# beer-asr/beer

Hardware: AMD Instinct MI355X
Metric: frames/sec per VB iteration (E+M) (higher is better)
Workload: dtype f32

## Files before the change

### beer_amd/csrc/estep_bf16.hip

```cpp

#include <cstdlib>
#include <type_traits>
#include <utility>

#include "estep_mfma.h"
#include "estep_tiles.h"

#ifndef BEER_K1_ABL
#define BEER_K1_ABL 0
#endif
#ifndef BEER_K2_ABL
#define BEER_K2_ABL 0
#endif
#ifndef BEER_AF_ABL
#define BEER_AF_ABL 0
#endif
#ifndef BEER_AFI_ABL
#define BEER_AFI_ABL 0
#endif
#ifndef BEER_LNFI_ABL
#define BEER_LNFI_ABL 0
#endif
#ifndef BEER_LNFI_SLEEP
#define BEER_LNFI_SLEEP 0
// ... 45 lines not shown
    else
        asm volatile("v_mfma_f32_16x16x32_bf16 %0, %1, %2, %0" : "+v"(acc) : "v"(a), "v"(b));
}
__device__ __forceinline__ void mfma_drain() {
    asm volatile("s_nop 15\n\ts_nop 15" ::: "memory");
    __builtin_amdgcn_sched_barrier(0);
}

__host__ __device__ inline size_t frame_image_tile_u4(int nk_used, int nqt) {
    return (size_t)(nk_used * NP * 2 + nqt * NP) * 64;
}
__host__ __device__ constexpr int img_nqt(int nk_used) { return nk_used <= 3 ? 5 : 6; }
constexpr int kImgMaxNK = 4;
__host__ __device__ inline int stat_slab(int j) { return j + j / 7; }
__host__ __device__ inline int nk16_of(int cov, int D) {
    return ((nslab_of(cov, D) + 7) / 8 + 1) / 2 * 2;
}
__host__ __device__ inline int ld16_of(int D) {
    const int ld = 4 * d4_of(D) + 8;
    return (ld / 4) % 2 ? ld : ld + 4;
}
constexpr float kConstEps = 5.9604644775390625e-8f;
constexpr int kBlockU4 = NP * 64;

__device__ inline double entry_value(int cov, int D, int K, int k, int slab, int e,
                                     const float* __restrict__ row, bool* is_const) {
    const int D4 = d4_of(D), Dp = 4 * D4, nslab = nslab_of(cov, D);
    *is_const = false;
    if (slab >= nslab) return 0.0;
    const int t = slab_entry(cov, D, slab);
    const int a = t & 0xff, b = ((t >> 8) & 0xff) + e, sq = t >> 16;
    if (a == Dp && b - e == Dp) {
        *is_const = true;
        return 0.0;
    }
    if (k >= K) return 0.0;
    if (sq) return b < D ? -0.5 * (double)row[cov == BEER_ISO ? D : D + b] : 0.0;
    if (a < D) {
        if (b >= D || b < a) return 0.0;
        return b == a ? -0.5 * (double)row[D + a * D + a]
                      : -0.5 * ((double)row[D + a * D + b] + (double)row[D + b * D + a]);
    }
    return b < D ? (double)row[b] : 0.0;
}
// ... 15 lines not shown

__global__ __launch_bounds__(256) void packx_kernel(int cov, int D, int K, int NT,
                                                    const float* __restrict__ E,
                                                    const float* __restrict__ logw,
                                                    unsigned short* __restrict__ P,
                                                    int* __restrict__ tab, int G, int Gp,
                                                    const float* __restrict__ c0, int lane_major) {
    extern __shared__ __attribute__((aligned(16))) char pack_lds[];
    const int nk = nk16_of(cov, D), nent = nk * 32;
    const int slot = blockIdx.x;
    const int k = slot % Gp < G ? (slot / Gp) * G + slot % Gp : K;
    const int chunk = slot / (NT * 16), kk = slot % (NT * 16);
    const int c = lane_major ? kk % NT : 4 * (kk / 64) + (kk % 4);
    const int i = lane_major ? kk / NT : (kk % 64) / 4;
    if (slot == 0)
        for (int s = threadIdx.x; s < (nk + 1) * 8; s += blockDim.x) {
            const int Dp = 4 * d4_of(D);
            tab[s] = s < nslab_of(cov, D) ? slab_entry(cov, D, s) : ((Dp + 2) | ((Dp + 4) << 8));
        }
    const int Qs = stats_dim(cov, D);
    float* rowl = reinterpret_cast<float*>(pack_lds);
    if (k < K)
        for (int q = threadIdx.x; q < Qs; q += blockDim.x) rowl[q] = E[(size_t)k * Qs + q];
    __syncthreads();
    unsigned short* base = P + ((size_t)chunk * nk * NT) * (NP * 512);
    auto put = [&](int q, float v) {
        const int s = q / 32, g = (q % 32) / 8, j = q % 8;
        unsigned short* dst = base + ((size_t)s * NT + c) * (NP * 512) + (g * 16 + i) * 8 + j;
        unsigned short p[3];
        split3_scalar(v, p);
        dst[0] = p[0];
        dst[512] = p[1];
        dst[1024] = p[2];
    };
    const int nslab = nslab_of(cov, D);
    for (int q = threadIdx.x; q < nent; q += blockDim.x) {
        bool is_const;
        const double v = entry_value(cov, D, K, k, q / 4, q % 4, rowl, &is_const);
        if (!is_const) {
            put(q, (float)v);
        } else if (q % 4 == 0) {
            const bool last = q / 4 == nslab - 1;
            const double want = k < K ? const_share(cov, D, q / 4, rowl, logw ? (double)logw[k] : 0.0) -
                                            (last ? (double)c0[0] : 0.0)
                                      : (last ? kPadLogit : 0.0);
            const float hi = (float)want;
            const double rem = (want - (double)hi) * (1.0 / (double)kConstEps);
            put(q, hi);
            put(q + 1, (rem == rem && fabs(rem) < 1.0e30) ? (float)rem : 0.f);
            put(q + 2, 0.f);
// ... 59 lines not shown
        }
    }
}

template <int NT, int MT, int GQ, bool PACKED, bool SQ, bool LNO, bool IMG = false, bool BL = false>
__global__ __launch_bounds__(kThreads, MT * NT <= 32 ? 2 : 1) void llhx_kernel(
    int64_t nframes, int D, int K, int S, int G, int gl, int jw, int nk,
    const float* __restrict__ X, const u4* __restrict__ Pall, const int* __restrict__ tab,
    float* __restrict__ resps, float* __restrict__ log_norm, double* __restrict__ llh_sum,
    float* __restrict__ xt_out, int xt_floats, int nku, int cg, const float* __restrict__ c0,
    const u4* __restrict__ img = nullptr) {
    static_assert(!IMG || (MT == 2 && !PACKED && LNO), "the image holds 32-frame tiles");
    static_assert(!BL || (NT == 16 && MT == 2 && !IMG), "half k-steps of 8 tiles, hipcc-scheduled form");
    extern __shared__ __attribute__((aligned(16))) char smem[];
    const int LD = ld16_of(D);
    const int tid = threadIdx.x, lane = tid & 63;
    const int wave = __builtin_amdgcn_readfirstlane(tid >> 6);
    const int i = lane & 15, g = lane >> 4;
    constexpr int FW = 16 * MT, NW = kThreads / 64;
    constexpr bool PIN = MT * NT > 32;
    float* xw = reinterpret_cast<float*>(smem) + wave * (FW * LD);
    int* tabs = reinterpret_cast<int*>(reinterpret_cast<float*>(smem) + NW * FW * LD);
    constexpr int kHalfBytes = 8 * kBlockU4 * 16;
    char* ring = smem + (((size_t)NW * FW * LD * sizeof(float) + (size_t)(nk + 1) * 8 * sizeof(int)
                          + 1023) & ~(size_t)1023);
    int64_t bx = blockIdx.x;
    int by = 0;
    {
        const int nch = (K + 16 * NT - 1) / (16 * NT);
        constexpr int FBK = FW * NW;
// ... 29 lines not shown
    for (int m = 0; m < MT; ++m)
#pragma unroll
        for (int c = 0; c < NT; ++c) acc[m][c] = f32x4{0, 0, 0, 0};

    const float* xrow[MT];
#pragma unroll
    for (int m = 0; m < MT; ++m) xrow[m] = xw + (m * 16 + i) * LD;

    const int kbase = by * (16 * NT);
    const u4* Pl = Pall + (size_t)by * nk * NT * kBlockU4 + lane;
    const int* tl = tabs + 2 * g;

    struct AFrag { u4 w[NP][MT]; };
    auto make_half = [&](int s, int m, int h, AFrag& f) {
        const int t = tl[8 * s + h];
        const int a = t & 0xff, j = (t >> 8) & 0xff;
        const bool sq = SQ && (t >> 16) != 0;
        const f32x4 bb = *reinterpret_cast<const f32x4*>(xrow[m] + j);
        const float xx = xrow[m][a];
        f32x4 p;
#pragma unroll
        for (int e = 0; e < 4; ++e) p[e] = bb[e] * (sq ? bb[e] : xx);
#pragma unroll
        for (int e = 0; e < 2; ++e) {
            unsigned w3[3];
            split3(p[2 * e], p[2 * e + 1], w3);
#pragma unroll
            for (int q = 0; q < NP; ++q) f.w[q][m][2 * h + e] = w3[q];
        }
    };
    constexpr int BT = 2, NBATCH = NT / BT;
    static_assert(NT % BT == 0 && NBATCH % 2 == 0, "B batches alternate between two buffers");
    struct BFrag { u4 p[BT][NP]; };
    auto load_b = [&](int64_t blk, BFrag& b) {
#pragma unroll
        for (int c = 0; c < BT; ++c)
#pragma unroll
// ... 17 lines not shown
#pragma unroll
        for (int n = 0; n < kHalfBytes / 1024 / NW; ++n)
            __builtin_amdgcn_global_load_lds(reinterpret_cast<const u4*>(src + n * (NW * 1024)),
                                             (lds_ptr)(dst + n * (NW * 1024)), 16, 0, 0);
    };
    auto publish = [&]() {
        asm volatile("s_waitcnt vmcnt(0) lgkmcnt(0)" ::: "memory");
        __builtin_amdgcn_s_barrier();
    };
    auto batch = [&](int s, int bi, const AFrag& cur, AFrag& nxt, const BFrag& b, BFrag& bn) {
        if constexpr (PIN) {
            static_assert(!PIN || (MT * 2 == NBATCH && 6 * BT * MT == 48), "one half fragment per batch");
            const int hm = bi % MT, hh = bi / MT;
            const int64_t blk = (int64_t)s * NT + (bi + 1) * BT;
            int t = 0;
            f32x4 bb = {0.f, 0.f, 0.f, 0.f}, p = {0.f, 0.f, 0.f, 0.f};
            float xx = 0.f;
            Split3Steps st[2];
#pragma unroll
            for (int n = 0; n < 48; ++n) {
                const int pr = n / (BT * MT), c = (n / MT) % BT, m = n % MT;
                mfma_bf16_pinned<false>(acc[m][bi * BT + c], cur.w[kProdA[pr]][m],
                                        b.p[c][kProdB[pr]]);
                if (BEER_K1_ABL >= 1 && n >= NP * BT) {
                } else if (BEER_K1_ABL >= 2) {
                } else if (n < NP * BT) {
#ifdef BEER_K1_FAKEB
                    bn.p[n / NP][n % NP] = Pl[(size_t)((blk + n / NP) & 3) * kBlockU4 + 64 * (n % NP)];
#else
                    bn.p[n / NP][n % NP] = Pl[(size_t)(blk + n / NP) * kBlockU4 + 64 * (n % NP)];
#endif
                } else if (n == 8) {
                    t = tl[8 * (s + 1) + hh];
                } else if (n == 12) {
                    bb = *reinterpret_cast<const f32x4*>(xrow[hm] + ((t >> 8) & 0xff));
                    xx = xrow[hm][t & 0xff];
                } else if (n >= 18 && n < 22) {
                    const bool sq = SQ && (t >> 16) != 0;
                    float v = bb[n - 18] * (sq ? bb[n - 18] : xx);
                    pin(v);
                    p[n - 18] = v;
                } else if (n >= 22 && n < 29) {
                    split3_step(n - 22, p[0], p[1], st[0]);
                } else if (n >= 29 && n < 36) {
                    split3_step(n - 29, p[2], p[3], st[1]);
                }
                if (BEER_K1_FENCE > 0 && n % BEER_K1_FENCE == BEER_K1_FENCE - 1)
                    __builtin_amdgcn_sched_barrier(0);
            }
            if (BEER_K1_ABL >= 1) {
#pragma unroll
                for (int q = 0; q < NP; ++q) nxt.w[q][hm] = cur.w[q][hm];
                if (BEER_K1_ABL >= 2) bn = b;
                return;
// ... 109 lines not shown
inline bool k1_lds_fits(int D, int nk) {
    size_t lds = (size_t)32 * (kThreads / 64) * ld16_of(D) * sizeof(float) + (size_t)(nk + 1) * 8 * sizeof(int);
    lds = ((lds + 1023) & ~(size_t)1023) + 2 * (size_t)(8 * kBlockU4 * 16);
    return 2 * lds <= (size_t)beer::kMaxDynLds;
}

thread_local int g_cov_of_launch = BEER_FULL;

template <int NT, int MT, int GQ, bool PACKED = false, bool SQ = true, bool LNO = false,
          bool IMG = false, bool BL = false>
int launch_llhx(int64_t nframes, int D, int K, int S, int G, int gl, int jw, int nchunks, int nk,
                const float* X, const void* P, const int* tab, const float* c0, float* resps,
                float* log_norm, double* llh_sum, hipStream_t s, float* xt_out = nullptr,
                int xt_floats = 0, const void* img = nullptr) {
    const int LD = ld16_of(D);
    const int nku = (nslab_of(SQ ? g_cov_of_launch : BEER_FULL, D) + 7) / 8;
    constexpr int FB = 16 * MT * (kThreads / 64);
    size_t lds = (size_t)FB * LD * sizeof(float) + (size_t)(nk + 1) * 8 * sizeof(int);
    if (BL) lds = ((lds + 1023) & ~(size_t)1023) + 2 * (size_t)(8 * kBlockU4 * 16);
    const int64_t blocks = (nframes + FB - 1) / FB;
    if (nchunks != (K + 16 * NT - 1) / (16 * NT)) return BEER_EINVAL;
    const int cg = xcd_chunk_group(nchunks, (size_t)nku * NT * kBlockU4 * 16);
    (void)hipFuncSetAttribute(
        reinterpret_cast<const void*>(llhx_kernel<NT, MT, GQ, PACKED, SQ, LNO, IMG, BL>),
        hipFuncAttributeMaxDynamicSharedMemorySize, beer::kMaxDynLds);
    hipLaunchKernelGGL((llhx_kernel<NT, MT, GQ, PACKED, SQ, LNO, IMG, BL>),
                       dim3(nchunks > 1 ? xcd_grid(blocks, nchunks, cg) : (unsigned)blocks),
                       dim3(kThreads), lds, s, nframes, D, K, S, G, gl, jw, nk, X,
                       reinterpret_cast<const u4*>(P), tab, resps, log_norm, llh_sum, xt_out,
                       xt_floats, nku, cg, c0, reinterpret_cast<const u4*>(img));
    BEER_LAUNCH_CHECK();
    return BEER_OK;
}

constexpr int kAxFT = 64;
constexpr int kAxXS = kAxFT + 4;
constexpr int kPiece = 4096;
constexpr int kAxMC = 8, kAxNQ = 8, kAxWaves = 4;

inline int xt_rows(int D) { return D + 2; }
inline int xt_pieces(int D) { return (xt_rows(D) * kAxXS * 4 + kPiece - 1) / kPiece; }

__global__ __launch_bounds__(256) void xt_image_kernel(int64_t nframes, int D, int NX,
                                                       const float* __restrict__ X,
                                                       float* __restrict__ Xt) {
    constexpr int LD = kMaxDimX + 1;
    __shared__ float tile[kAxFT * LD];
    const int64_t tau = blockIdx.x, t0 = tau * kAxFT;
    const int rows = (int)(nframes - t0 < kAxFT ? nframes - t0 : kAxFT);
    for (int e = threadIdx.x; e < rows * D; e += 256) {
        const int f = e / D, d = e - f * D;
        tile[f * LD + d] = X[t0 * D + e];
    }
    __syncthreads();
    float* out = Xt + tau * ((size_t)NX * (kPiece / 4));
    for (int e = threadIdx.x; e < NX * (kPiece / 4); e += 256) {
        const int row = e / kAxXS, col = e - row * kAxXS;
        float v = 0.f;
        if (row < D) v = col < rows ? tile[col * LD + row] : 0.f;
        else if (row == D) v = 1.f;
        __builtin_nontemporal_store(v, out + e);
    }
}

template <bool SR>
__global__ __launch_bounds__(64 * kAxWaves, 1) void accx_kernel(
    int64_t nframes, int D, int K, int nslab, int NX, const float* __restrict__ Xt,
    const unsigned* __restrict__ Rimg, const int* __restrict__ tab,
    int64_t frames_per_block, double* __restrict__ Sp, int gx, int gy, int gz,
    const float* __restrict__ Gt, int lgG, int sx) {
    constexpr int MC = kAxMC, NQ = kAxNQ, WAVES = kAxWaves, NB = 2;
    static_assert(16 * MC == kPackedComps && kAxFT == kPackedFrames, "the packed image is this kernel's LDS tile");
    constexpr int plane = kPackedPlaneWords * 4;
    const int r_off = NX * kPiece, buf_bytes = r_off + NP * plane;
    const int xstride = sx ? 0 : buf_bytes;
    const int rstride = sx ? NP * plane : buf_bytes;
    const int g_base = sx ? r_off + NB * NP * plane : NB * buf_bytes;
    extern __shared__ __attribute__((aligned(16))) char smem[];
    const int tid = threadIdx.x, lane = tid & 63;
    const int wave = __builtin_amdgcn_readfirstlane(tid >> 6);
    const int i = lane & 15, g = lane >> 4;
    const int D4 = d4_of(D), Dp = 4 * D4, nq = nslab * 4;
    const int id = blockIdx.x, xcd = id & 7, slot0 = id >> 3;
    const int bx = slot0 % gx;
    const int yz = (slot0 / gx) * 8 + xcd;
    if (yz >= gy * gz) return;
// ... 1 lines not shown
    const int tile0 = (bx * WAVES + wave) * NQ;
    const int kc0 = by * (16 * MC);
    const int64_t tb = (int64_t)bz * frames_per_block;
    const int64_t te = tb + frames_per_block < nframes ? tb + frames_per_block : nframes;
    const int ntiles = (int)((te - tb + kAxFT - 1) / kAxFT);
    const int64_t tau0 = tb / kAxFT;
    const int nblk = (K + 16 * MC - 1) / (16 * MC);
    const int gbytes = SR ? ((16 * MC) >> lgG) * kAxFT * 4 : 0;
    const int gkb = (gbytes + 1023) >> 10;

    auto factors = [&](int uu, int& a, int& b) {
        const int col = 16 * (tile0 + uu) + i, slab = col >> 2;
        a = b = Dp + 2;
        if (slab < nslab) {
            const int t = tab[slab];
            b = ((t >> 8) & 0xff) + (col & 3);
            a = (t >> 16) ? b : (t & 0xff);
        }
    };
    int xa_off[NQ], xb_off[NQ];
#pragma unroll
    for (int uu = 0; uu < NQ; ++uu) {
        int a, b;
        factors(uu, a, b);
        xa_off[uu] = ((a < D ? a : (a == Dp ? D : D + 1)) * kAxXS + 8 * g) * 4;
        xb_off[uu] = ((b < D ? b : (b == Dp ? D : D + 1)) * kAxXS + 8 * g) * 4;
    }
    int a_off[kAxFT / 32];
#pragma unroll
    for (int ks = 0; ks < kAxFT / 32; ++ks)
        a_off[ks] = r_off + (i * kPackedFrames + (((4 * ks + g) ^ (i & 7)) << 3)) * 2;

// ... 104 lines not shown
#pragma unroll
            for (int q = 0; q < NP; ++q) out[q][e] = w3[q];
        }
    };
    if (active && ntiles > 0) gen_b(0, 0, 0, bf[0]);
    auto iteration = [&](int tile, int buf) __attribute__((always_inline)) {
        const int next = buf ^ 1;
        if (tile + 1 < ntiles) stage(tile + 1, next);
        const bool fold_next = SR && tile + 1 < ntiles;
        if (active) {
#pragma unroll
            for (int ks = 0; ks < 2; ++ks) {
                if (BEER_K2_ABL < 2 || (tile == 0 && ks == 0)) load_a(buf, ks);
#pragma unroll
                for (int uu = 0; uu < NQ; ++uu) {
                    const int cur = uu & 1;
                    const bool build = BEER_K2_ABL < 1 && (uu + 1 < NQ || ks == 0);
                    const int nks = uu + 1 < NQ ? ks : 1, nuu = uu + 1 < NQ ? uu + 1 : 0;
                    const char* pa = smem + xa_off[nuu] + (buf * xstride + 128 * nks);
                    const char* pb = smem + xb_off[nuu] + (buf * xstride + 128 * nks);
                    f32x4 xa[2], xb[2];
                    float pp[8];
                    Split3Steps st[4];
#pragma unroll
                    for (int n = 0; n < 6 * MC; ++n) {
                        const int pr = n / MC, c = n % MC;
                        mfma_bf16_pinned<false>(acc[c][uu], af[c][kPA[pr]], bf[cur][kPB[pr]]);
                        if (!build) continue;
                        if (n == 1) xa[0] = *reinterpret_cast<const f32x4*>(pa);
                        else if (n == 2) xa[1] = *reinterpret_cast<const f32x4*>(pa + 16);
                        else if (n == 3) xb[0] = *reinterpret_cast<const f32x4*>(pb);
// ... 993 lines not shown

inline int group_pad(int G) {
    int p = 1;
    while (p < G) p <<= 1;
    return p;
}
inline int accf_group_pad(int S, int G) { return (G + 3) / 4 * 4; }
inline bool supported_llh_padded(int D, int S, int G) {
    return supported_llh_x(D, S, S > 1 ? group_pad(G) : G);
}

inline int ntx_for(int S, int K) { return S > 1 ? 16 : (K <= 64 ? 4 : (K <= 128 ? 8 : 16)); }
inline int nchunksx_for(int S, int K) { return S > 1 ? (K + 255) / 256 : 1; }
size_t up256(size_t n) { return (n + 255) / 256 * 256; }

inline size_t p_image_bytes(int nchunks, int nk, int NT) {
    return up256(((size_t)nchunks * nk * NT + 4) * kBlockU4 * 16);
}

}

#ifdef BEER_KERNEL_PROBE
namespace {
template __global__ void llhx_kernel<16, 4, 4, true, false, false>(
    int64_t, int, int, int, int, int, int, int, const float*, const u4*, const int*, float*, float*,
    double*, float*, int, int, int, const float*, const u4*);
template __global__ void llhx_kernel<16, 2, 1, false, true, true>(
    int64_t, int, int, int, int, int, int, int, const float*, const u4*, const int*, float*, float*,
    double*, float*, int, int, int, const float*, const u4*);
template __global__ void llhx_kernel<16, 2, 1, false, true, true, true>(
    int64_t, int, int, int, int, int, int, int, const float*, const u4*, const int*, float*, float*,
    double*, float*, int, int, int, const float*, const u4*);
template __global__ void accx_kernel<false>(int64_t, int, int, int, int, const float*, const unsigned*,
                                            const int*, int64_t, double*, int, int, int,
                                            const float*, int, int);
template __global__ void accx_kernel<true>(int64_t, int, int, int, int, const float*, const unsigned*,
                                           const int*, int64_t, double*, int, int, int,
                                           const float*, int, int);
template __global__ void lnfi_kernel<3, 16>(int64_t, int, int, int, const u4*, const u4*, float*, double*,
                                            int64_t, const float*);
template __global__ void accfi_kernel<3, 8>(int64_t, int, int, int, int, int, int, const u4*, const u4*,
                                         const float*, const float*, int64_t, double*, const float*);
template __global__ void accf_kernel<4, 6, true, 8, 5, true>(int64_t, int, int, int, int, int, int, int,
                                                       const float*, const u4*, const int*,
                                                       const float*, const float*, int64_t, double*,
                                                       const float*);
}
#else
bool supported_llh_split(int D, int S, int G) { return supported_llh_padded(D, S, G); }
bool supported_llh_packed_sets(int cov, int D, int S, int G) {
    return cov == BEER_FULL && S > 1 && G >= 4 && G <= 128 && (G & (G - 1)) == 0 &&
           supported_llh_padded(D, S, G) && supported_acc_x(D, S * G);
}
// ... 191 lines not shown
            case 1: BEER_LLHX(16, 2, 1, false, true);
            case 2: BEER_LLHX(16, 2, 2, false, true);
            default: BEER_LLHX(16, 2, 4, false, true);
        }
    }
    switch (gq) {
        case 1: BEER_LLHX(16, 2, 1, false, false);
        case 2: BEER_LLHX(16, 2, 2, false, false);
        default: BEER_LLHX(16, 2, 4, false, false);
    }
#undef BEER_LLHX
}

size_t accx_base_workspace_bytes(int cov, int D, int K) {
    if (!supported_acc_x(D, K)) return 0;
    const int nslab = nslab_of(cov, D);
    return up256((size_t)K * nslab * 4 * sizeof(double)) + up256((size_t)nslab * sizeof(int)) + 1024;
}

size_t accx_workspace_bytes(int cov, int64_t nframes, int D, int K) {
    const size_t base = accx_base_workspace_bytes(cov, D, K);
    if (base == 0) return 0;
    const int64_t tiles = (nframes + kAxFT - 1) / kAxFT;
    return base + (size_t)tiles * xt_pieces(D) * kPiece;
}

bool supported_acc_sets(int cov, int D, int S, int G) {
    return S >= 1 && G >= 8 && G <= 128 && (G & (G - 1)) == 0 && supported_acc_x(D, S * G);
}
inline int acc_sets_spad(int S, int G) {
    return (S * G + kPackedComps - 1) / kPackedComps * (kPackedComps / G);
// ... 1 lines not shown
size_t accxs_workspace_bytes(int cov, int64_t nframes, int D, int S, int G) {
    if (!supported_acc_sets(cov, D, S, G)) return 0;
    const int64_t tiles = (nframes + kAxFT - 1) / kAxFT;
    return up256(accx_workspace_bytes(cov, nframes, D, S * G)) +
           (size_t)tiles * acc_sets_spad(S, G) * kAxFT * sizeof(float) + 1024;
}

int acc_bf16x3_packed(int cov, int64_t nframes, int D, int K, const float* X, const void* Rimg,
                      double* acc, void* ws, size_t ws_bytes, hipStream_t s, int S, int G,
                      const float* SR) {
    if (!supported_acc_x(D, K) || ws_bytes < accx_workspace_bytes(cov, nframes, D, K))
        return BEER_EINVAL;
    if (SR && (S * G != K || !supported_acc_sets(cov, D, S, G) ||
               ws_bytes < accxs_workspace_bytes(cov, nframes, D, S, G)))
        return BEER_EINVAL;
    const int nslab = nslab_of(cov, D), nq = nslab * 4;
    char* w = reinterpret_cast<char*>(ws);
    double* Sp = reinterpret_cast<double*>(w);
    w += up256((size_t)K * nq * sizeof(double));
    int* tab = reinterpret_cast<int*>(w);
    float* Xt = reinterpret_cast<float*>(reinterpret_cast<char*>(ws) +
                                         accx_base_workspace_bytes(cov, D, K));
    hipError_t e = hipMemsetAsync(Sp, 0, (size_t)K * nq * sizeof(double), s);
    if (e != hipSuccess) return -(int)e;
    hipLaunchKernelGGL(tab_kernel, dim3(1), dim3(256), 0, s, cov, D, tab);
    BEER_LAUNCH_CHECK();
    const int64_t tiles = (nframes + kAxFT - 1) / kAxFT;
    const int NX = xt_pieces(D);
    if (packed_has_xt(K) && !SR) {
        Xt = reinterpret_cast<float*>(const_cast<char*>(reinterpret_cast<const char*>(Rimg)) +
                                      packed_tiles_bytes(nframes, K));
    } else {
        hipLaunchKernelGGL(xt_image_kernel, dim3((unsigned)tiles), dim3(256), 0, s, nframes, D, NX,
                           X, Xt);
        BEER_LAUNCH_CHECK();
    }
    const int ntiles = (nq + 15) / 16;
    float* Gt = nullptr;
    int lgG = 0;
    if (SR) {
        Gt = reinterpret_cast<float*>(reinterpret_cast<char*>(ws) +
                                      up256(accx_workspace_bytes(cov, nframes, D, K)));
        const int spad = acc_sets_spad(S, G);
        hipLaunchKernelGGL(gt_image_kernel, dim3((unsigned)tiles, (unsigned)((spad + 63) / 64)),
                           dim3(256), 0, s, nframes, S, spad, SR, Gt);
        BEER_LAUNCH_CHECK();
        while ((1 << lgG) < G) ++lgG;
    }
    const int gx = (ntiles + kAxNQ * kAxWaves - 1) / (kAxNQ * kAxWaves);
    const int gy = (K + 16 * kAxMC - 1) / (16 * kAxMC);
    const int chain = beer::option(BEER_OPT_AX_MAXFRAMES);
    const int64_t max_z = (nframes + 511) / 512, min_z = (nframes + chain - 1) / chain;
    const int64_t rounds = ((int64_t)gx * gy * min_z + 255) / 256;
    int64_t gz = rounds * 256 / ((int64_t)gx * gy);
    if (gz < min_z) gz = min_z;
    if (gz > max_z) gz = max_z;
    if (gz < 1) gz = 1;
    int64_t fpb = (nframes + gz - 1) / gz;
    fpb = (fpb + kAxFT - 1) / kAxFT * kAxFT;
    gz = (nframes + fpb - 1) / fpb;
    size_t lds = 2 * ((size_t)NX * kPiece + (size_t)NP * kPackedPlaneWords * 4) +
                 (SR ? 2 * 4096 : 0);
    const int sx = lds > (size_t)beer::kMaxDynLds ? 1 : 0;
    if (sx) lds = (size_t)NX * kPiece + 2 * (size_t)NP * kPackedPlaneWords * 4 + (SR ? 2 * 4096 : 0);
    const int64_t nyz = ((int64_t)gy * gz + 7) / 8 * 8;
    const dim3 grid((unsigned)(nyz * gx));
#define BEER_ACCX(SR_)                                                                           \
    do {                                                                                         \
        (void)hipFuncSetAttribute(reinterpret_cast<const void*>(accx_kernel<SR_>),               \
                                  hipFuncAttributeMaxDynamicSharedMemorySize, beer::kMaxDynLds);         \
        hipLaunchKernelGGL((accx_kernel<SR_>), grid, dim3(64 * kAxWaves), lds, s, nframes, D, K, \
                           nslab, NX, Xt, reinterpret_cast<const unsigned*>(Rimg), tab, fpb, Sp, \
                           gx, gy, (int)gz, Gt, lgG, sx);                                        \
    } while (0)
    if (SR) BEER_ACCX(true);
    else BEER_ACCX(false);
#undef BEER_ACCX
    BEER_LAUNCH_CHECK();
    const int64_t total = (int64_t)K * stats_dim(cov, D);
    hipLaunchKernelGGL(unpack_kernel, dim3((unsigned)((total + 255) / 256)), dim3(256), 0, s, cov,
                       D, K, Sp, acc);
    BEER_LAUNCH_CHECK();
    return BEER_OK;
}

bool supported_accf(int cov, int D, int S, int G) {
    return cov != BEER_FULL && D >= 1 && D <= 64 && S >= 1 && G >= 1 && G <= 256 &&
           nslab_of(cov, D) * 4 <= 160;
}

size_t accf_workspace_bytes(int cov, int D, int S, int G) {
    if (!supported_accf(cov, D, S, G)) return 0;
    const int Kreal = S * G;
    G = accf_group_pad(S, G);
    const int K = S * G, NTC = accf_ntc(cov, D), nk = nk16_of(cov, D);
// ... 2 lines not shown
           up256((size_t)Kreal * nq * sizeof(double));
}

bool supported_frame_image(int cov, int D) {
    if (cov == BEER_FULL || D < 1) return false;
    const int nk_used = (nslab_of(cov, D) + 7) / 8;
    return nk_used <= kImgMaxNK && 2 * d4_of(D) <= 4 * img_nqt(nk_used);
}
size_t frame_image_bytes(int cov, int64_t nframes, int D) {
    if (!supported_frame_image(cov, D) || nframes < 0) return 0;
    const int nk = nk16_of(cov, D), nk_used = (nslab_of(cov, D) + 7) / 8;
    const int64_t tiles = (nframes + 31) / 32;
    return (size_t)tiles * frame_image_tile_u4(nk_used, img_nqt(nk_used)) * 16 +
           up256((size_t)(nk + 1) * 8 * sizeof(int));
}
__global__ void tabx_kernel(int cov, int D, int nk, int* __restrict__ tab) {
    const int Dp = 4 * d4_of(D);
    for (int s = threadIdx.x; s < (nk + 1) * 8; s += blockDim.x)
        tab[s] = s < nslab_of(cov, D) ? slab_entry(cov, D, s) : ((Dp + 2) | ((Dp + 4) << 8));
}
int frame_image(int cov, int64_t nframes, int D, const float* X, void* image, hipStream_t s) {
    if (!supported_frame_image(cov, D)) return BEER_EINVAL;
    if (nframes == 0) return BEER_OK;
    const int nk = nk16_of(cov, D), nslab = nslab_of(cov, D), nk_used = (nslab + 7) / 8;
    const int64_t tiles = (nframes + 31) / 32;
    int* tab = reinterpret_cast<int*>(reinterpret_cast<char*>(image) +
                                      (size_t)tiles * frame_image_tile_u4(nk_used, img_nqt(nk_used)) * 16);
    hipLaunchKernelGGL(tabx_kernel, dim3(1), dim3(256), 0, s, cov, D, nk, tab);
    const size_t lds = (size_t)(nk + 1) * 8 * sizeof(int) +
                       (size_t)4 * (32 * ld16_of(D) + (D + 2) * kAfXS) * sizeof(float);
    hipLaunchKernelGGL(frame_image_kernel, dim3((unsigned)((tiles + 3) / 4)), dim3(256), lds, s,
                       nframes, D, nk, nslab, img_nqt(nk_used), X, tab, reinterpret_cast<u4*>(image));
    BEER_LAUNCH_CHECK();
    return BEER_OK;
}

int acc_fused_bf16x3(int cov, int64_t nframes, int D, int S, int G, const float* X,
                     const float* expT, const float* logw, const float* log_norm,
                     const float* sr, const void* image, double* acc, void* ws, size_t ws_bytes,
                     hipStream_t s) {
    if (!supported_accf(cov, D, S, G) || ws_bytes < accf_workspace_bytes(cov, D, S, G))
        return BEER_EINVAL;
    const int Greal = G, Kreal = S * G;
// ... 57 lines not shown
        hipLaunchKernelGGL((accfi_kernel<NKU_, W_, NS_>), grid, dim3(64 * W_), lds_f, s, nframes, \
                           K, S, G, Greal, nk, nslab, reinterpret_cast<const u4*>(image),        \
                           reinterpret_cast<const u4*>(P), log_norm, sr, fpb, Sp, c0);           \
    } while (0)
#define BEER_ACCFI_K(W_, NS_)                                                                    \
    do {                                                                                         \
        if (nk_used == 1) BEER_ACCFI(1, W_, NS_); else if (nk_used == 2) BEER_ACCFI(2, W_, NS_); \
        else if (nk_used == 3) BEER_ACCFI(3, W_, NS_); else BEER_ACCFI(4, W_, NS_);              \
    } while (0)
        if (waves == 8) { if (ns_img == 4) BEER_ACCFI_K(8, 4); else BEER_ACCFI_K(8, 16); }
        else { if (ns_img == 4) BEER_ACCFI_K(4, 4); else BEER_ACCFI_K(4, 16); }
#undef BEER_ACCFI_K
#undef BEER_ACCFI
        BEER_LAUNCH_CHECK();
        const int64_t total_i = (int64_t)Kreal * stats_dim(cov, D);
        hipLaunchKernelGGL(unpack_kernel, dim3((unsigned)((total_i + 255) / 256)), dim3(256), 0, s,
                           cov, D, Kreal, Sp, acc);
        BEER_LAUNCH_CHECK();
        return BEER_OK;
    }
#define BEER_ACCF(NTC_, NQT_, W_, BLK_)                                                          \
    do {                                                                                         \
        constexpr int XP_ = NQT_ == 6 ? 5 : 8;             \
        (void)hipFuncSetAttribute(                                                               \
            reinterpret_cast<const void*>(accf_kernel<NTC_, NQT_, true, W_, XP_, BLK_>),         \
            hipFuncAttributeMaxDynamicSharedMemorySize, beer::kMaxDynLds);                               \
        hipLaunchKernelGGL((accf_kernel<NTC_, NQT_, true, W_, XP_, BLK_>), grid, dim3(64 * W_),  \
                           lds, s, nframes, D, K, S, G, Greal, nk, nslab, X,                     \
                           reinterpret_cast<const u4*>(P), tab, log_norm, sr, fpb, Sp, c0);      \
    } while (0)
    if (NQT == 6) { if (blk) BEER_ACCF(4, 6, 8, true); else BEER_ACCF(4, 6, 8, false); }
    else if (NQT == 9) { if (blk) BEER_ACCF(4, 9, 4, true); else BEER_ACCF(4, 9, 4, false); }
    else { if (blk) BEER_ACCF(4, 10, 4, true); else BEER_ACCF(4, 10, 4, false); }
#undef BEER_ACCF
    BEER_LAUNCH_CHECK();
    const int64_t total = (int64_t)Kreal * stats_dim(cov, D);
    hipLaunchKernelGGL(unpack_kernel, dim3((unsigned)((total + 255) / 256)), dim3(256), 0, s, cov,
                       D, Kreal, Sp, acc);
    BEER_LAUNCH_CHECK();
    return BEER_OK;
}

#endif

}
```

### beer_amd/csrc/estep_tiles.h

```cpp
#pragma once
#include <type_traits>

#include <hip/hip_runtime.h>

#include "common.h"

namespace beer_mfma {

using namespace beer;

typedef float f32x4 __attribute__((ext_vector_type(4)));
typedef double f64x4 __attribute__((ext_vector_type(4)));

#ifndef BEER_EXP_VALU
#define BEER_EXP_VALU 0
#endif
#ifndef BEER_LNFI_TRANS_EVERY
#define BEER_LNFI_TRANS_EVERY 0
#endif
__device__ __forceinline__ float exp2_valu(float y) {
    if (!BEER_EXP_VALU) return __builtin_amdgcn_exp2f(y);
    y = __builtin_fmaxf(y, -125.f);
    const float magic = 12582912.f;
    const float t = y + magic;
// ... 110 lines not shown
        const int nslab = nslab_of(cov, D);
        if (a >= D && j >= D4) return nslab - 1;
        const int want = a >= D ? 1 : 0;
        for (int s = 0; s < nslab; ++s) {
            int k, q;
            diag_walk(D, s, &k, &q);
            if (k == want && q == j) return s;
        }
        return nslab - 1;
    }
    if (a >= D) return nslab_of(cov, D) - (D4 + 1) + j;
    const int q = a / 4, r = a % 4;
    const int before = 4 * (q * D4 - q * (q - 1) / 2) + r * (D4 - q);
    return before + (j - q);
}
template <typename T>
__host__ __device__ inline double const_total(int cov, int D, const T* row, double logw) {
    const int Q = stats_dim(cov, D);
    const double zero = cov == BEER_ISO ? 0.5 * (double)D : 0.5;
    return -0.5 * (double)row[Q - 2] + zero * (double)row[Q - 1] - 0.5 * (double)D * kLog2Pi + logw;
}
template <typename T>
__host__ __device__ inline double const_share(int cov, int D, int slab, const T* row, double logw) {
    const double total = const_total(cov, D, row, logw);
    if (cov == BEER_FULL) return total;
    double given = 0.0, pending = 0.0;
    const int nslab = nslab_of(cov, D);
    for (int s = 0; s < nslab; ++s) {
        int k, q;
        diag_walk(D, s, &k, &q);
// ... 14 lines not shown
__host__ __device__ inline int nslab_padded(int cov, int D) {
    return (nslab_of(cov, D) + 1) / 2 * 2 + 1;
}

constexpr int kThreads = 256;
constexpr double kPadLogit = -1.0e30;

namespace {

__global__ void tab_kernel(int cov, int D, int* __restrict__ tab) {
    const int nslab = nslab_of(cov, D);
    for (int s = blockIdx.x * blockDim.x + threadIdx.x; s < nslab; s += gridDim.x * blockDim.x)
        tab[s] = slab_entry(cov, D, s);
}

__global__ void unpack_kernel(int cov, int D, int K, const double* __restrict__ Sp,
                              double* __restrict__ acc) {
    const int D4 = d4_of(D), Dp = 4 * D4, nq = nslab_of(cov, D) * 4;
    const int Q = stats_dim(cov, D);
    const int64_t total = (int64_t)K * Q;
    for (int64_t idx = (int64_t)blockIdx.x * blockDim.x + threadIdx.x; idx < total;
         idx += (int64_t)gridDim.x * blockDim.x) {
        const int k = (int)(idx / Q), q = (int)(idx % Q);
        const double* s = Sp + (size_t)k * nq;
        double v;
        if (q < D) {
            v = s[slab_index(cov, D, Dp, q / 4) * 4 + q % 4];
        } else if (q >= Q - 2) {
            const double n = s[slab_index(cov, D, Dp, D4) * 4];
            v = (q == Q - 2) ? -0.5 * n : (cov == BEER_ISO ? 0.5 * (double)D * n : 0.5 * n);
        } else if (cov == BEER_FULL) {
            int a = (q - D) / D, b = (q - D) % D;
            if (a > b) { const int t = a; a = b; b = t; }
            v = -0.5 * s[slab_index(cov, D, a, b / 4) * 4 + b % 4];
        } else if (cov == BEER_DIAG) {
            const int d = q - D;
            v = -0.5 * s[slab_index(cov, D, d, d / 4) * 4 + d % 4];
        } else {
            double tot = 0.0;
            for (int d = 0; d < D; ++d) tot += s[slab_index(cov, D, d, d / 4) * 4 + d % 4];
            v = -0.5 * tot;
        }
        acc[idx] += v;
    }
}

}

constexpr int kPackedFrames = 64, kPackedComps = 128, kPackedPieces = 3;
constexpr int kPackedPlaneWords = kPackedComps * kPackedFrames / 2;

__host__ __device__ inline size_t packed_word(int64_t tau, int nblk, int beta, int kk, int f6) {
    const int half = kk * kPackedFrames + (((f6 >> 3) ^ (kk & 7)) << 3) + (f6 & 7);
    return ((size_t)tau * nblk + beta) * (kPackedPieces * kPackedPlaneWords) + (half >> 1);
}

__device__ __forceinline__ unsigned cvt_pk_bf16(float a, float b) {
    typedef __bf16 bf2_t __attribute__((ext_vector_type(2)));
    typedef float f2_t __attribute__((ext_vector_type(2)));
// ... 334 lines not shown
```

Before: 235.1 million.

## Use diagonal-band slab layout for full-covariance second-order statistics

For full covariance, the upper-triangular slab enumeration of x·xᵀ products is replaced by a cyclic diagonal band layout. Each slab now holds four products x[a+e]·x[(a+e+d) mod Dp], which packs the symmetric matrix with fewer padded slabs. The layout change runs through packing, the llh and accumulation kernels, the table builder and the unpack step. The accumulation kernel's per-wave tile count NQ also becomes a template parameter chosen from 6 to 8 to reduce tail waste. The cost is gathered, per-element column reads in place of one broadcast value, and more template instantiations.

```diff
diff --git a/beer_amd/csrc/estep_bf16.hip b/beer_amd/csrc/estep_bf16.hip
--- a/beer_amd/csrc/estep_bf16.hip
+++ b/beer_amd/csrc/estep_bf16.hip
@@ -83,7 +83,7 @@
 constexpr int kImgMaxNK = 4;
 __host__ __device__ inline int stat_slab(int j) { return j + j / 7; }
 __host__ __device__ inline int nk16_of(int cov, int D) {
-    return ((nslab_of(cov, D) + 7) / 8 + 1) / 2 * 2;
+    return ((nslabx_of(cov, D) + 7) / 8 + 1) / 2 * 2;
 }
 __host__ __device__ inline int ld16_of(int D) {
     const int ld = 4 * d4_of(D) + 8;
@@ -94,9 +94,25 @@
 
 __device__ inline double entry_value(int cov, int D, int K, int k, int slab, int e,
                                      const float* __restrict__ row, bool* is_const) {
-    const int D4 = d4_of(D), Dp = 4 * D4, nslab = nslab_of(cov, D);
+    const int D4 = d4_of(D), Dp = 4 * D4, nslab = nslabx_of(cov, D);
     *is_const = false;
     if (slab >= nslab) return 0.0;
+    if (band_layout(cov, D)) {
+        const int nb = band_nslab(D);
+        if (slab == nslab - 1) {
+            *is_const = true;
+            return 0.0;
+        }
+        if (k >= K) return 0.0;
+        if (slab >= nb) {
+            const int b = 4 * (slab - nb) + e;
+            return b < D ? (double)row[b] : 0.0;
+        }
+        int a, b;
+        if (!band_pair(D, slab, e, &a, &b)) return 0.0;
+        return b == a ? -0.5 * (double)row[D + a * D + a]
+                      : -0.5 * ((double)row[D + a * D + b] + (double)row[D + b * D + a]);
+    }
     const int t = slab_entry(cov, D, slab);
     const int a = t & 0xff, b = ((t >> 8) & 0xff) + e, sq = t >> 16;
     if (a == Dp && b - e == Dp) {
@@ -142,10 +158,7 @@
     const int c = lane_major ? kk % NT : 4 * (kk / 64) + (kk % 4);
     const int i = lane_major ? kk / NT : (kk % 64) / 4;
     if (slot == 0)
-        for (int s = threadIdx.x; s < (nk + 1) * 8; s += blockDim.x) {
-            const int Dp = 4 * d4_of(D);
-            tab[s] = s < nslab_of(cov, D) ? slab_entry(cov, D, s) : ((Dp + 2) | ((Dp + 4) << 8));
-        }
+        for (int s = threadIdx.x; s < (nk + 1) * 8; s += blockDim.x) tab[s] = slabx_entry(cov, D, s);
     const int Qs = stats_dim(cov, D);
     float* rowl = reinterpret_cast<float*>(pack_lds);
     if (k < K)
@@ -161,7 +174,7 @@
         dst[512] = p[1];
         dst[1024] = p[2];
     };
-    const int nslab = nslab_of(cov, D);
+    const int nslab = nslabx_of(cov, D);
     for (int q = threadIdx.x; q < nent; q += blockDim.x) {
         bool is_const;
         const double v = entry_value(cov, D, K, k, q / 4, q % 4, rowl, &is_const);
@@ -251,6 +264,7 @@
     static_assert(!BL || (NT == 16 && MT == 2 && !IMG), "half k-steps of 8 tiles, hipcc-scheduled form");
     extern __shared__ __attribute__((aligned(16))) char smem[];
     const int LD = ld16_of(D);
+    const int Dp = 4 * d4_of(D);
     const int tid = threadIdx.x, lane = tid & 63;
     const int wave = __builtin_amdgcn_readfirstlane(tid >> 6);
     const int i = lane & 15, g = lane >> 4;
@@ -310,13 +324,19 @@
     struct AFrag { u4 w[NP][MT]; };
     auto make_half = [&](int s, int m, int h, AFrag& f) {
         const int t = tl[8 * s + h];
-        const int a = t & 0xff, j = (t >> 8) & 0xff;
-        const bool sq = SQ && (t >> 16) != 0;
-        const f32x4 bb = *reinterpret_cast<const f32x4*>(xrow[m] + j);
-        const float xx = xrow[m][a];
         f32x4 p;
-#pragma unroll
-        for (int e = 0; e < 4; ++e) p[e] = bb[e] * (sq ? bb[e] : xx);
+        if constexpr (SQ) {
+            const int a = t & 0xff, j = (t >> 8) & 0xff;
+            const bool sq = (t >> 16) != 0;
+            const f32x4 bb = *reinterpret_cast<const f32x4*>(xrow[m] + j);
+            const float xx = xrow[m][a];
+#pragma unroll
+            for (int e = 0; e < 4; ++e) p[e] = bb[e] * (sq ? bb[e] : xx);
+        } else {
+            const f32x4 bb = *reinterpret_cast<const f32x4*>(xrow[m] + (t & 0xff));
+#pragma unroll
+            for (int e = 0; e < 4; ++e) p[e] = bb[e] * xrow[m][band_col(t, e, Dp)];
+        }
 #pragma unroll
         for (int e = 0; e < 2; ++e) {
             unsigned w3[3];
@@ -364,7 +384,7 @@
             const int hm = bi % MT, hh = bi / MT;
             const int64_t blk = (int64_t)s * NT + (bi + 1) * BT;
             int t = 0;
-            f32x4 bb = {0.f, 0.f, 0.f, 0.f}, p = {0.f, 0.f, 0.f, 0.f};
+            f32x4 bb = {0.f, 0.f, 0.f, 0.f}, p = {0.f, 0.f, 0.f, 0.f}, yy = {0.f, 0.f, 0.f, 0.f};
             float xx = 0.f;
             Split3Steps st[2];
 #pragma unroll
@@ -383,11 +403,13 @@
                 } else if (n == 8) {
                     t = tl[8 * (s + 1) + hh];
                 } else if (n == 12) {
-                    bb = *reinterpret_cast<const f32x4*>(xrow[hm] + ((t >> 8) & 0xff));
-                    xx = xrow[hm][t & 0xff];
+                    bb = *reinterpret_cast<const f32x4*>(xrow[hm] + (SQ ? (t >> 8) & 0xff : t & 0xff));
+                    if (SQ) xx = xrow[hm][t & 0xff];
+                } else if (!SQ && n >= 13 && n < 17) {
+                    yy[n - 13] = xrow[hm][band_col(t, n - 13, Dp)];
                 } else if (n >= 18 && n < 22) {
                     const bool sq = SQ && (t >> 16) != 0;
-                    float v = bb[n - 18] * (sq ? bb[n - 18] : xx);
+                    float v = bb[n - 18] * (SQ ? (sq ? bb[n - 18] : xx) : yy[n - 18]);
                     pin(v);
                     p[n - 18] = v;
                 } else if (n >= 22 && n < 29) {
@@ -527,7 +549,7 @@
                 float* log_norm, double* llh_sum, hipStream_t s, float* xt_out = nullptr,
                 int xt_floats = 0, const void* img = nullptr) {
     const int LD = ld16_of(D);
-    const int nku = (nslab_of(SQ ? g_cov_of_launch : BEER_FULL, D) + 7) / 8;
+    const int nku = (nslabx_of(SQ ? g_cov_of_launch : BEER_FULL, D) + 7) / 8;
     constexpr int FB = 16 * MT * (kThreads / 64);
     size_t lds = (size_t)FB * LD * sizeof(float) + (size_t)(nk + 1) * 8 * sizeof(int);
     if (BL) lds = ((lds + 1023) & ~(size_t)1023) + 2 * (size_t)(8 * kBlockU4 * 16);
@@ -549,7 +571,7 @@
 constexpr int kAxFT = 64;
 constexpr int kAxXS = kAxFT + 4;
 constexpr int kPiece = 4096;
-constexpr int kAxMC = 8, kAxNQ = 8, kAxWaves = 4;
+constexpr int kAxMC = 8, kAxWaves = 4;
 
 inline int xt_rows(int D) { return D + 2; }
 inline int xt_pieces(int D) { return (xt_rows(D) * kAxXS * 4 + kPiece - 1) / kPiece; }
@@ -576,13 +598,13 @@
     }
 }
 
-template <bool SR>
+template <bool SR, int NQ>
 __global__ __launch_bounds__(64 * kAxWaves, 1) void accx_kernel(
     int64_t nframes, int D, int K, int nslab, int NX, const float* __restrict__ Xt,
     const unsigned* __restrict__ Rimg, const int* __restrict__ tab,
     int64_t frames_per_block, double* __restrict__ Sp, int gx, int gy, int gz,
-    const float* __restrict__ Gt, int lgG, int sx) {
-    constexpr int MC = kAxMC, NQ = kAxNQ, WAVES = kAxWaves, NB = 2;
+    const float* __restrict__ Gt, int lgG, int sx, int band) {
+    constexpr int MC = kAxMC, WAVES = kAxWaves, NB = 2;
     static_assert(16 * MC == kPackedComps && kAxFT == kPackedFrames, "the packed image is this kernel's LDS tile");
     constexpr int plane = kPackedPlaneWords * 4;
     const int r_off = NX * kPiece, buf_bytes = r_off + NP * plane;
@@ -614,8 +636,13 @@
         a = b = Dp + 2;
         if (slab < nslab) {
             const int t = tab[slab];
-            b = ((t >> 8) & 0xff) + (col & 3);
-            a = (t >> 16) ? b : (t & 0xff);
+            if (band) {
+                a = (t & 0xff) + (col & 3);
+                b = band_col(t, col & 3, Dp);
+            } else {
+                b = ((t >> 8) & 0xff) + (col & 3);
+                a = (t >> 16) ? b : (t & 0xff);
+            }
         }
     };
     int xa_off[NQ], xb_off[NQ];
@@ -750,7 +777,7 @@
                 if (BEER_K2_ABL < 2 || (tile == 0 && ks == 0)) load_a(buf, ks);
 #pragma unroll
                 for (int uu = 0; uu < NQ; ++uu) {
-                    const int cur = uu & 1;
+                    const int cur = (ks * NQ + uu) & 1;
                     const bool build = BEER_K2_ABL < 1 && (uu + 1 < NQ || ks == 0);
                     const int nks = uu + 1 < NQ ? ks : 1, nuu = uu + 1 < NQ ? uu + 1 : 0;
                     const char* pa = smem + xa_off[nuu] + (buf * xstride + 128 * nks);
@@ -1774,6 +1801,15 @@
 inline int nchunksx_for(int S, int K) { return S > 1 ? (K + 255) / 256 : 1; }
 size_t up256(size_t n) { return (n + 255) / 256 * 256; }
 
+inline int accx_nq(int ntiles) {
+    int best = 0, cost = 0;
+    for (int nq = 8; nq >= 6; --nq) {
+        const int c = (ntiles + kAxWaves * nq - 1) / (kAxWaves * nq) * nq;
+        if (best == 0 || c < cost) { cost = c; best = nq; }
+    }
+    return best;
+}
+
 inline size_t p_image_bytes(int nchunks, int nk, int NT) {
     return up256(((size_t)nchunks * nk * NT + 4) * kBlockU4 * 16);
 }
@@ -1783,6 +1819,9 @@
 #ifdef BEER_KERNEL_PROBE
 namespace {
 template __global__ void llhx_kernel<16, 4, 4, true, false, false>(
+    int64_t, int, int, int, int, int, int, int, const float*, const u4*, const int*, float*, float*,
+    double*, float*, int, int, int, const float*, const u4*);
+template __global__ void llhx_kernel<16, 2, 4, true, false, false, false, true>(
     int64_t, int, int, int, int, int, int, int, const float*, const u4*, const int*, float*, float*,
     double*, float*, int, int, int, const float*, const u4*);
 template __global__ void llhx_kernel<16, 2, 1, false, true, true>(
@@ -1791,12 +1830,12 @@
 template __global__ void llhx_kernel<16, 2, 1, false, true, true, true>(
     int64_t, int, int, int, int, int, int, int, const float*, const u4*, const int*, float*, float*,
     double*, float*, int, int, int, const float*, const u4*);
-template __global__ void accx_kernel<false>(int64_t, int, int, int, int, const float*, const unsigned*,
-                                            const int*, int64_t, double*, int, int, int,
-                                            const float*, int, int);
-template __global__ void accx_kernel<true>(int64_t, int, int, int, int, const float*, const unsigned*,
-                                           const int*, int64_t, double*, int, int, int,
-                                           const float*, int, int);
+template __global__ void accx_kernel<false, 7>(int64_t, int, int, int, int, const float*, const unsigned*,
+                                               const int*, int64_t, double*, int, int, int,
+                                               const float*, int, int, int);
+template __global__ void accx_kernel<true, 7>(int64_t, int, int, int, int, const float*, const unsigned*,
+                                              const int*, int64_t, double*, int, int, int,
+                                              const float*, int, int, int);
 template __global__ void lnfi_kernel<3, 16>(int64_t, int, int, int, const u4*, const u4*, float*, double*,
                                             int64_t, const float*);
 template __global__ void accfi_kernel<3, 8>(int64_t, int, int, int, int, int, int, const u4*, const u4*,
@@ -2018,7 +2057,7 @@
 
 size_t accx_base_workspace_bytes(int cov, int D, int K) {
     if (!supported_acc_x(D, K)) return 0;
-    const int nslab = nslab_of(cov, D);
+    const int nslab = nslabx_of(cov, D);
     return up256((size_t)K * nslab * 4 * sizeof(double)) + up256((size_t)nslab * sizeof(int)) + 1024;
 }
 
@@ -2050,7 +2089,7 @@
     if (SR && (S * G != K || !supported_acc_sets(cov, D, S, G) ||
                ws_bytes < accxs_workspace_bytes(cov, nframes, D, S, G)))
         return BEER_EINVAL;
-    const int nslab = nslab_of(cov, D), nq = nslab * 4;
+    const int nslab = nslabx_of(cov, D), nq = nslab * 4;
     char* w = reinterpret_cast<char*>(ws);
     double* Sp = reinterpret_cast<double*>(w);
     w += up256((size_t)K * nq * sizeof(double));
@@ -2059,7 +2098,7 @@
                                          accx_base_workspace_bytes(cov, D, K));
     hipError_t e = hipMemsetAsync(Sp, 0, (size_t)K * nq * sizeof(double), s);
     if (e != hipSuccess) return -(int)e;
-    hipLaunchKernelGGL(tab_kernel, dim3(1), dim3(256), 0, s, cov, D, tab);
+    hipLaunchKernelGGL(tabx_kernel, dim3(1), dim3(256), 0, s, cov, D, nslab, tab);
     BEER_LAUNCH_CHECK();
     const int64_t tiles = (nframes + kAxFT - 1) / kAxFT;
     const int NX = xt_pieces(D);
@@ -2083,7 +2122,8 @@
         BEER_LAUNCH_CHECK();
         while ((1 << lgG) < G) ++lgG;
     }
-    const int gx = (ntiles + kAxNQ * kAxWaves - 1) / (kAxNQ * kAxWaves);
+    const int NQ = accx_nq(ntiles);
+    const int gx = (ntiles + NQ * kAxWaves - 1) / (NQ * kAxWaves);
     const int gy = (K + 16 * kAxMC - 1) / (16 * kAxMC);
     const int chain = beer::option(BEER_OPT_AX_MAXFRAMES);
     const int64_t max_z = (nframes + 511) / 512, min_z = (nframes + chain - 1) / chain;
@@ -2101,20 +2141,27 @@
     if (sx) lds = (size_t)NX * kPiece + 2 * (size_t)NP * kPackedPlaneWords * 4 + (SR ? 2 * 4096 : 0);
     const int64_t nyz = ((int64_t)gy * gz + 7) / 8 * 8;
     const dim3 grid((unsigned)(nyz * gx));
-#define BEER_ACCX(SR_)                                                                           \
+    const int band = band_layout(cov, D) ? 1 : 0;
+#define BEER_ACCX(SR_, NQ_)                                                                      \
     do {                                                                                         \
-        (void)hipFuncSetAttribute(reinterpret_cast<const void*>(accx_kernel<SR_>),               \
-                                  hipFuncAttributeMaxDynamicSharedMemorySize, beer::kMaxDynLds);         \
-        hipLaunchKernelGGL((accx_kernel<SR_>), grid, dim3(64 * kAxWaves), lds, s, nframes, D, K, \
-                           nslab, NX, Xt, reinterpret_cast<const unsigned*>(Rimg), tab, fpb, Sp, \
-                           gx, gy, (int)gz, Gt, lgG, sx);                                        \
+        (void)hipFuncSetAttribute(reinterpret_cast<const void*>(accx_kernel<SR_, NQ_>),          \
+                                  hipFuncAttributeMaxDynamicSharedMemorySize, beer::kMaxDynLds); \
+        hipLaunchKernelGGL((accx_kernel<SR_, NQ_>), grid, dim3(64 * kAxWaves), lds, s, nframes, \
+                           D, K, nslab, NX, Xt, reinterpret_cast<const unsigned*>(Rimg), tab,    \
+                           fpb, Sp, gx, gy, (int)gz, Gt, lgG, sx, band);                         \
     } while (0)
-    if (SR) BEER_ACCX(true);
-    else BEER_ACCX(false);
+#define BEER_ACCX_NQ(SR_)                                                                        \
+    do {                                                                                         \
+        if (NQ == 6) BEER_ACCX(SR_, 6); else if (NQ == 7) BEER_ACCX(SR_, 7);                     \
+        else BEER_ACCX(SR_, 8);                                                                  \
+    } while (0)
+    if (SR) BEER_ACCX_NQ(true);
+    else BEER_ACCX_NQ(false);
+#undef BEER_ACCX_NQ
 #undef BEER_ACCX
     BEER_LAUNCH_CHECK();
     const int64_t total = (int64_t)K * stats_dim(cov, D);
-    hipLaunchKernelGGL(unpack_kernel, dim3((unsigned)((total + 255) / 256)), dim3(256), 0, s, cov,
+    hipLaunchKernelGGL(unpackx_kernel, dim3((unsigned)((total + 255) / 256)), dim3(256), 0, s, cov,
                        D, K, Sp, acc);
     BEER_LAUNCH_CHECK();
     return BEER_OK;
@@ -2147,11 +2194,6 @@
     return (size_t)tiles * frame_image_tile_u4(nk_used, img_nqt(nk_used)) * 16 +
            up256((size_t)(nk + 1) * 8 * sizeof(int));
 }
-__global__ void tabx_kernel(int cov, int D, int nk, int* __restrict__ tab) {
-    const int Dp = 4 * d4_of(D);
-    for (int s = threadIdx.x; s < (nk + 1) * 8; s += blockDim.x)
-        tab[s] = s < nslab_of(cov, D) ? slab_entry(cov, D, s) : ((Dp + 2) | ((Dp + 4) << 8));
-}
 int frame_image(int cov, int64_t nframes, int D, const float* X, void* image, hipStream_t s) {
     if (!supported_frame_image(cov, D)) return BEER_EINVAL;
     if (nframes == 0) return BEER_OK;
@@ -2159,7 +2201,7 @@
     const int64_t tiles = (nframes + 31) / 32;
     int* tab = reinterpret_cast<int*>(reinterpret_cast<char*>(image) +
                                       (size_t)tiles * frame_image_tile_u4(nk_used, img_nqt(nk_used)) * 16);
-    hipLaunchKernelGGL(tabx_kernel, dim3(1), dim3(256), 0, s, cov, D, nk, tab);
+    hipLaunchKernelGGL(tabx_kernel, dim3(1), dim3(256), 0, s, cov, D, (nk + 1) * 8, tab);
     const size_t lds = (size_t)(nk + 1) * 8 * sizeof(int) +
                        (size_t)4 * (32 * ld16_of(D) + (D + 2) * kAfXS) * sizeof(float);
     hipLaunchKernelGGL(frame_image_kernel, dim3((unsigned)((tiles + 3) / 4)), dim3(256), lds, s,
@@ -2247,7 +2289,7 @@
 #undef BEER_ACCFI
         BEER_LAUNCH_CHECK();
         const int64_t total_i = (int64_t)Kreal * stats_dim(cov, D);
-        hipLaunchKernelGGL(unpack_kernel, dim3((unsigned)((total_i + 255) / 256)), dim3(256), 0, s,
+        hipLaunchKernelGGL(unpackx_kernel, dim3((unsigned)((total_i + 255) / 256)), dim3(256), 0, s,
                            cov, D, Kreal, Sp, acc);
         BEER_LAUNCH_CHECK();
         return BEER_OK;
@@ -2268,7 +2310,7 @@
 #undef BEER_ACCF
     BEER_LAUNCH_CHECK();
     const int64_t total = (int64_t)Kreal * stats_dim(cov, D);
-    hipLaunchKernelGGL(unpack_kernel, dim3((unsigned)((total + 255) / 256)), dim3(256), 0, s, cov,
+    hipLaunchKernelGGL(unpackx_kernel, dim3((unsigned)((total + 255) / 256)), dim3(256), 0, s, cov,
                        D, Kreal, Sp, acc);
     BEER_LAUNCH_CHECK();
     return BEER_OK;
diff --git a/beer_amd/csrc/estep_tiles.h b/beer_amd/csrc/estep_tiles.h
--- a/beer_amd/csrc/estep_tiles.h
+++ b/beer_amd/csrc/estep_tiles.h
@@ -148,6 +148,64 @@
     const int before = 4 * (q * D4 - q * (q - 1) / 2) + r * (D4 - q);
     return before + (j - q);
 }
+__host__ __device__ inline bool band_layout(int cov, int D) { return cov == BEER_FULL; }
+__host__ __device__ inline int band_nslab(int D) {
+    const int Dp = 4 * d4_of(D), h = Dp / 2;
+    return h * (Dp / 4) + (h + 3) / 4;
+}
+__host__ __device__ inline int band_entry(int D, int s) {
+    const int D4 = d4_of(D), Dp = 4 * D4, nb = band_nslab(D);
+    if (s < nb) {
+        const int d = s / D4, a4 = 4 * (s - d * D4);
+        return a4 | (1 << 8) | ((a4 + d) << 16);
+    }
+    if (s < nb + D4) return (4 * (s - nb)) | ((2 * Dp) << 16);
+    if (s == nb + D4) return Dp | ((2 * Dp) << 16);
+    return (Dp + 4) | ((2 * Dp + 2) << 16);
+}
+__host__ __device__ __forceinline__ int band_col(int t, int e, int Dp) {
+    const unsigned c = (unsigned)((t >> 16) + ((t >> 8) & 1) * e), w = c - (unsigned)Dp;
+    return (int)(w < c ? w : c);
+}
+__host__ __device__ inline int band_pos(int D, int a, int b) {
+    const int D4 = d4_of(D), Dp = 4 * D4;
+    if (a > b) { const int t = a; a = b; b = t; }
+    int d = b - a, start = a;
+    if (2 * d > Dp) { d = Dp - d; start = b; }
+    return 4 * (d * D4 + start / 4) + start % 4;
+}
+__host__ __device__ inline bool band_pair(int D, int s, int e, int* a, int* b) {
+    const int D4 = d4_of(D), Dp = 4 * D4;
+    const int d = s / D4;
+    *a = 4 * (s - d * D4) + e;
+    *b = (*a + d) % Dp;
+    if (*a >= D || *b >= D) return false;
+    return !(2 * d == Dp && 2 * *a >= Dp);
+}
+
+__host__ __device__ inline int nslabx_of(int cov, int D) {
+    return band_layout(cov, D) ? band_nslab(D) + d4_of(D) + 1 : nslab_of(cov, D);
+}
+__host__ __device__ inline int slabx_entry(int cov, int D, int s) {
+    if (band_layout(cov, D)) return band_entry(D, s);
+    const int Dp = 4 * d4_of(D);
+    return s < nslab_of(cov, D) ? slab_entry(cov, D, s) : ((Dp + 2) | ((Dp + 4) << 8));
+}
+__host__ __device__ inline int slab_pos(int cov, int D, int a, int b) {
+    const int D4 = d4_of(D), Dp = 4 * D4;
+    if (a < 0) return slab_index(cov, D, Dp, D4) * 4;
+    if (b < 0) return slab_index(cov, D, Dp, a / 4) * 4 + a % 4;
+    if (a > b) { const int t = a; a = b; b = t; }
+    return slab_index(cov, D, a, b / 4) * 4 + b % 4;
+}
+__host__ __device__ inline int slabx_pos(int cov, int D, int a, int b) {
+    if (!band_layout(cov, D)) return slab_pos(cov, D, a, b);
+    const int D4 = d4_of(D), nb = band_nslab(D);
+    if (a < 0) return 4 * (nb + D4);
+    if (b < 0) return 4 * nb + a;
+    return band_pos(D, a, b);
+}
+
 template <typename T>
 __host__ __device__ inline double const_total(int cov, int D, const T* row, double logw) {
     const int Q = stats_dim(cov, D);
@@ -192,10 +250,15 @@
         tab[s] = slab_entry(cov, D, s);
 }
 
-__global__ void unpack_kernel(int cov, int D, int K, const double* __restrict__ Sp,
-                              double* __restrict__ acc) {
-    const int D4 = d4_of(D), Dp = 4 * D4, nq = nslab_of(cov, D) * 4;
+template <bool BAND>
+__device__ inline void unpack_stats(int cov, int D, int K, const double* __restrict__ Sp,
+                                    double* __restrict__ acc) {
+    const bool band = BAND && band_layout(cov, D);
+    const int nq = (band ? nslabx_of(cov, D) : nslab_of(cov, D)) * 4;
     const int Q = stats_dim(cov, D);
+    auto pos = [&](int a, int b) {
+        return band ? slabx_pos(cov, D, a, b) : slab_pos(cov, D, a, b);
+    };
     const int64_t total = (int64_t)K * Q;
     for (int64_t idx = (int64_t)blockIdx.x * blockDim.x + threadIdx.x; idx < total;
          idx += (int64_t)gridDim.x * blockDim.x) {
@@ -203,24 +266,33 @@
         const double* s = Sp + (size_t)k * nq;
         double v;
         if (q < D) {
-            v = s[slab_index(cov, D, Dp, q / 4) * 4 + q % 4];
+            v = s[pos(q, -1)];
         } else if (q >= Q - 2) {
-            const double n = s[slab_index(cov, D, Dp, D4) * 4];
+            const double n = s[pos(-1, 0)];
             v = (q == Q - 2) ? -0.5 * n : (cov == BEER_ISO ? 0.5 * (double)D * n : 0.5 * n);
         } else if (cov == BEER_FULL) {
-            int a = (q - D) / D, b = (q - D) % D;
-            if (a > b) { const int t = a; a = b; b = t; }
-            v = -0.5 * s[slab_index(cov, D, a, b / 4) * 4 + b % 4];
+            v = -0.5 * s[pos((q - D) / D, (q - D) % D)];
         } else if (cov == BEER_DIAG) {
-            const int d = q - D;
-            v = -0.5 * s[slab_index(cov, D, d, d / 4) * 4 + d % 4];
+            v = -0.5 * s[pos(q - D, q - D)];
         } else {
             double tot = 0.0;
-            for (int d = 0; d < D; ++d) tot += s[slab_index(cov, D, d, d / 4) * 4 + d % 4];
+            for (int d = 0; d < D; ++d) tot += s[pos(d, d)];
             v = -0.5 * tot;
         }
         acc[idx] += v;
     }
+}
+__global__ void unpack_kernel(int cov, int D, int K, const double* __restrict__ Sp,
+                              double* __restrict__ acc) {
+    unpack_stats<false>(cov, D, K, Sp, acc);
+}
+__global__ void unpackx_kernel(int cov, int D, int K, const double* __restrict__ Sp,
+                               double* __restrict__ acc) {
+    unpack_stats<true>(cov, D, K, Sp, acc);
+}
+__global__ void tabx_kernel(int cov, int D, int n, int* __restrict__ tab) {
+    for (int s = blockIdx.x * blockDim.x + threadIdx.x; s < n; s += gridDim.x * blockDim.x)
+        tab[s] = slabx_entry(cov, D, s);
 }
 
 }
```

New measurement: 252.6 million (median of 6 runs). 1.07x the previous value.
